# Zialus/CUDA-Recommender

Hardware: AMD Instinct MI355X
Metric: rating-nnz/sec per CCD++ outer iter at k=64 (higher is better)
Workload: dtype f32

## Files before the change

cuda-recommender_amd/csrc/ccd_kernels.hip:

```cpp
#include "ccd_kernels.hpp"

#include <algorithm>
#include <cstdlib>
#include <mutex>
#include <type_traits>

#include "flat_layout.hpp"

namespace mfx {
namespace {

constexpr int kBlock = 256;
constexpr uint32_t kPerSegLdsCap = 1024;

using u32x4 = __attribute__((ext_vector_type(4))) uint32_t;
using f32x4 = __attribute__((ext_vector_type(4))) float;
using u16x4 = __attribute__((ext_vector_type(4))) uint16_t;

template <int CTRL, int ROW_MASK = 0xF>
__device__ __forceinline__ float dpp_mov(float src) {
    return __builtin_bit_cast(float, __builtin_amdgcn_update_dpp(0, __builtin_bit_cast(int, src), CTRL, ROW_MASK, 0xF, true));
}
constexpr int kDppRowShr = 0x110, kDppWaveShr1 = 0x138, kDppBcast15 = 0x142, kDppBcast31 = 0x143;

// ... 111 lines not shown
    const uint32_t* orphans;
    uint32_t norphans, ngroups, panel_lanes;
    uint32_t nseg, npanels;
    const uint32_t* ptr_v;
    const uint32_t* rank_code;
    const uint32_t* seg_cnt;
    float lambda;
    float* out_vec;
    float2* pack2;
    const float* next_vec;
    float4* pack4;
    const float* gather_aux;
};

struct F3 { float x, y, z; };
template <typename S, typename G> __device__ __forceinline__ S to_slice(const G& g) { return g; }
template <> __device__ __forceinline__ F3 to_slice<F3, float4>(const float4& g) { return F3{g.x, g.y, g.z}; }
template <typename G, typename S> __device__ __forceinline__ G from_slice(const S& s) { return s; }
template <> __device__ __forceinline__ float4 from_slice<float4, F3>(const F3& s) { return make_float4(s.x, s.y, s.z, 0.f); }
template <int MODE> struct ModeTraits;
template <> struct ModeTraits<FM_SWEEP> { using G = float;  using S = float;  using P = float;  static constexpr bool kPerSeg = false, kWrite = false, kDot = true, kAux = false; };
template <> struct ModeTraits<FM_RESID> { using G = float;  using S = float;  using P = float;  static constexpr bool kPerSeg = true,  kWrite = true,  kDot = false, kAux = false; };
template <> struct ModeTraits<FM_FCSC>  { using G = float2; using S = float2; using P = float2; static constexpr bool kPerSeg = true,  kWrite = true,  kDot = true, kAux = false; };
template <> struct ModeTraits<FM_FCSR>  { using G = float4; using S = F3;     using P = float2; static constexpr bool kPerSeg = true,  kWrite = true,  kDot = true, kAux = false; };
template <> struct ModeTraits<FM_FCSC_RO> { using G = float2; using S = float2; using P = float2; static constexpr bool kPerSeg = true, kWrite = false, kDot = true, kAux = false; };
template <> struct ModeTraits<FM_FCSR_RO> { using G = float4; using S = F3;     using P = float2; static constexpr bool kPerSeg = true, kWrite = false, kDot = true, kAux = false; };
template <> struct ModeTraits<FM_FCSC2> { using G = float4; using S = float4; using P = float4; static constexpr bool kPerSeg = true,  kWrite = true,  kDot = true, kAux = false; };
template <> struct ModeTraits<FM_FCSR2> { using G = float4; using S = float4; using P = float4; static constexpr bool kPerSeg = true,  kWrite = true,  kDot = true, kAux = true; };

__device__ __forceinline__ float zero_of(float) { return 0.f; }
__device__ __forceinline__ float2 zero_of(float2) { return make_float2(0.f, 0.f); }
__device__ __forceinline__ float4 zero_of(float4) { return make_float4(0.f, 0.f, 0.f, 0.f); }

template <int MODE>
__device__ __forceinline__ void element_op(float v, const typename ModeTraits<MODE>::G& ga, float aux,
                                           const typename ModeTraits<MODE>::P& ps, int add,
                                           float& v_out, float& gc, float& hc) {
    if constexpr (MODE == FM_SWEEP) {
        v_out = v;
        gc = ga * v;
        hc = ga * ga;
    } else if constexpr (MODE == FM_RESID) {
        const float prod = mul_rn(ga, ps);
        v_out = add ? add_rn(v, prod) : sub_rn(v, prod);
        gc = 0.f;
        hc = 0.f;
    } else if constexpr (MODE == FM_FCSC || MODE == FM_FCSC_RO) {
        v_out = add_rn(sub_rn(v, mul_rn(ga.x, ps.x)), mul_rn(ga.y, ps.y));
        gc = ga.y * v_out;
        hc = ga.y * ga.y;
    } else if constexpr (MODE == FM_FCSR || MODE == FM_FCSR_RO) {
        v_out = add_rn(sub_rn(v, mul_rn(ga.x, ps.x)), mul_rn(ga.y, ps.y));
        gc = ga.z * v_out;
        hc = ga.z * ga.z;
    } else {
        const float r = add_rn(sub_rn(v, mul_rn(ga.x, ps.x)), mul_rn(ga.y, ps.y));
        v_out = add_rn(sub_rn(r, mul_rn(ga.z, ps.z)), mul_rn(ga.w, ps.w));
        const float d = MODE == FM_FCSC2 ? ga.w : aux;
        gc = d * v_out;
        hc = d * d;
    }
}

template <int BLOCK> __device__ void fused_finalize(const FlatArgs& a, uint32_t chunk, unsigned char* lds_raw);

using gu64 = __attribute__((address_space(1))) unsigned long long;
using gu32 = __attribute__((address_space(1))) uint32_t;
template <bool FUSE>
__device__ __forceinline__ void store_partial(float2* p, float g, float h) {
    if constexpr (FUSE) {
        const unsigned long long bits = (unsigned long long) __builtin_bit_cast(uint32_t, g) | ((unsigned long long) __builtin_bit_cast(uint32_t, h) << 32);
        __hip_atomic_store((gu64*) p, bits, __ATOMIC_RELAXED, __HIP_MEMORY_SCOPE_AGENT);
    } else {
        *p = make_float2(g, h);
    }
}
__device__ __forceinline__ float2 load_partial_sc1(const float2* p) {
    const unsigned long long bits = __hip_atomic_load((gu64*) p, __ATOMIC_RELAXED, __HIP_MEMORY_SCOPE_AGENT);
    return make_float2(__builtin_bit_cast(float, (uint32_t) bits), __builtin_bit_cast(float, (uint32_t) (bits >> 32)));
}

template <int MODE> constexpr int flat_min_waves(int block) { return MODE == FM_FCSC_RO || MODE == FM_FCSR_RO ? block / 128 : 1; }

template <int MODE, bool LDS, int BLOCK, bool PSCHK, bool FUSE = false, bool PERSIST = false>
__global__ __launch_bounds__(BLOCK, flat_min_waves<MODE>(BLOCK)) void k_flat(FlatArgs a) {
    static_assert(!FUSE || ModeTraits<MODE>::kDot, "fused finalize: passes that produce sums");
    static_assert(!PERSIST || (LDS && !FUSE), "persistent form: LDS panels without the in-pass finalize");
    using TR = ModeTraits<MODE>;
    uint32_t chunk = FUSE ? a.wg_order[blockIdx.x] : blockIdx.x;
    uint32_t chunk_end = chunk + 1;
    const uint32_t nchunks = a.nspans / (BLOCK / 64);
    if constexpr (PERSIST) {
        chunk = (uint32_t) ((uint64_t) blockIdx.x * nchunks / gridDim.x);
        chunk_end = (uint32_t) ((uint64_t) (blockIdx.x + 1) * nchunks / gridDim.x);
        if (chunk >= chunk_end) return;
    }
    using G = typename TR::G;
    using P = typename TR::P;
    extern __shared__ __attribute__((aligned(16))) unsigned char lds_raw[];
    using S = typename TR::S;
    S* __restrict__ slice = reinterpret_cast<S*>(lds_raw);
    constexpr size_t kSliceEntry = sizeof(S) + (TR::kAux ? sizeof(float) : 0);
    float* __restrict__ aux_slice = reinterpret_cast<float*>(lds_raw + ((size_t) a.panel_rows + 1) * sizeof(S));
    const uint32_t lane = threadIdx.x & 63;
    uint32_t span = __builtin_amdgcn_readfirstlane(chunk * (BLOCK / 64) + (threadIdx.x >> 6));
    const G* __restrict__ gather = static_cast<const G*>(a.gather);
    const P* __restrict__ perseg = static_cast<const P*>(a.perseg);
    const uint32_t span_words = a.tiles_per_span * (kTileElems / 32);
    uint64_t start = (uint64_t) span * a.tiles_per_span * kTileElems;
    using IdxVec = typename std::conditional<LDS, u16x4, u32x4>::type;
    using IdxElem = typename std::conditional<LDS, uint16_t, uint32_t>::type;
    const IdxVec* __restrict__ idx4 = reinterpret_cast<const IdxVec*>(static_cast<const IdxElem*>(a.idx) + start) + lane;
    f32x4* __restrict__ val4 = reinterpret_cast<f32x4*>(a.val + start) + lane;
    const uint32_t* __restrict__ flw = a.flags32 + (size_t) span * span_words + (lane >> 3);
    const uint32_t* __restrict__ hpw = a.hpre + (size_t) span * span_words + (lane >> 3);
    const uint32_t sh = (lane & 7) * 4;
    IdxVec id_n;
    f32x4 v_n;
    uint32_t fl_n, hp_n, hp_nn;
    const size_t span_step_q = (size_t) (BLOCK / 64) * a.tiles_per_span * 64, span_step_w = (size_t) (BLOCK / 64) * span_words;
    auto stage_slice = [&](uint32_t panel) {
        const uint32_t gbase = panel * a.panel_rows;
        const uint32_t cnt = a.gather_len - gbase < a.panel_rows ? a.gather_len - gbase : a.panel_rows;
        for (uint32_t i = threadIdx.x; i < cnt; i += BLOCK) slice[i] = to_slice<S, G>(gather[gbase + i]);
        if (threadIdx.x == 0) slice[a.panel_rows] = S{};
        if constexpr (TR::kAux) {
            for (uint32_t i = threadIdx.x; i < cnt; i += BLOCK) aux_slice[i] = a.gather_aux[gbase + i];
            if (threadIdx.x == 0) aux_slice[a.panel_rows] = 0.f;
        }
    };
    uint32_t panel = 0, panel_next = 0;
    if constexpr (LDS) {
        id_n = __builtin_nontemporal_load(idx4);
        v_n = __builtin_nontemporal_load(val4);
        fl_n = flw[0]; hp_n = hpw[0]; hp_nn = hpw[8];
        panel = a.wg_panel[chunk];
        stage_slice(panel);
    }
    P* __restrict__ ps_lds = reinterpret_cast<P*>(lds_raw + (((size_t) a.panel_rows + 1) * kSliceEntry + 15) / 16 * 16);
    uint32_t win_base = 0;
    auto heads_before = [&](uint32_t c) { return a.hpre[(size_t) c * (BLOCK / 64) * span_words]; };
    uint32_t hb1 = 0, hb2 = 0;
    if constexpr (LDS && TR::kPerSeg) {
        const uint32_t rb0 = heads_before(chunk);
        win_base = rb0 > 0 ? rb0 - 1 : 0;
        const uint32_t win_end = heads_before(chunk + 1);
        if constexpr (PERSIST) { hb1 = win_end; hb2 = heads_before(chunk + 2 < nchunks ? chunk + 2 : nchunks); }
        uint32_t cnt = win_end - win_base;
        if (cnt > kPerSegLdsCap) cnt = kPerSegLdsCap;
        for (uint32_t j = threadIdx.x; j < cnt; j += BLOCK) ps_lds[j] = perseg[a.seg_of_rank[win_base + j]];
    }
    if constexpr (LDS && !PERSIST) __syncthreads();
    for (uint32_t visit = 0;; ++visit) {
    const bool more = PERSIST && chunk + 1 < chunk_end;
    uint32_t win_base_n = 0, win_cnt_n = 0;
    if constexpr (PERSIST) {
        if (visit && panel_next != panel) {
            __syncthreads();
            panel = panel_next;
            stage_slice(panel);
        }
        __syncthreads();
        if constexpr (TR::kPerSeg) {
            if (more) {
                win_base_n = hb1 > 0 ? hb1 - 1 : 0;
                win_cnt_n = hb2 - win_base_n < kPerSegLdsCap ? hb2 - win_base_n : kPerSegLdsCap;
            }
        }
    }
    P* __restrict__ ps_cur = PERSIST ? ps_lds + (visit & 1u) * kPerSegLdsCap : ps_lds;
    bool live = span < a.nspans;
    if constexpr (!FUSE) { if (!live) return; }
    auto fetch_ps = [&](uint32_t r) -> P {
        if constexpr (LDS) {
            const uint32_t rl = r - win_base;
            if constexpr (!PSCHK) return ps_cur[rl];
            else if (rl < kPerSegLdsCap) return ps_cur[rl];
        }
        return perseg[a.seg_of_rank[r]];
    };
    uint32_t ntiles = a.tiles_per_span;
    if constexpr (!LDS) {
        const uint64_t left = a.nnz > start ? a.nnz - start : 0;
        const uint32_t nlive = (uint32_t) ((left + kTileElems - 1) / kTileElems);
        if (nlive < ntiles) ntiles = nlive;
        if (live && ntiles == 0) {
            if (TR::kDot && lane == 0) store_partial<FUSE>(a.carry + span, 0.f, 0.f);
            live = false;
        }
        if constexpr (!FUSE) { if (!live) return; }
        if (live) {
            id_n = __builtin_nontemporal_load(idx4);
            v_n = __builtin_nontemporal_load(val4);
            fl_n = flw[0]; hp_n = hpw[0]; hp_nn = hpw[8];
        }
    }
    if (live) {
    const uint32_t rank_base = __builtin_amdgcn_readfirstlane(hp_n);
    uint32_t cur1 = rank_base;
    P pcur{};
    if constexpr (TR::kPerSeg) {
        if (cur1 > 0) pcur = fetch_ps(cur1 - 1);
    }
    float og = 0.f, oh = 0.f;
    bool open_spread = false;

    for (uint32_t tile = 0; tile < ntiles; ++tile) {
        const IdxVec id = id_n;
        const f32x4 v = v_n;
        const uint32_t fl = fl_n, hp = hp_n;
        const uint32_t cur1_next = __builtin_amdgcn_readfirstlane(hp_nn);
        hp_n = hp_nn;
        if constexpr (!PERSIST) {
            if (tile + 1 < ntiles) {
                id_n = __builtin_nontemporal_load(idx4 + (tile + 1) * 64);
                v_n = __builtin_nontemporal_load(val4 + (tile + 1) * 64);
            }
            fl_n = flw[(tile + 1) * 8];
            hp_nn = hpw[(tile + 2) * 8];
        } else if (tile + 1 < ntiles) {
            id_n = __builtin_nontemporal_load(idx4 + (tile + 1) * 64);
            v_n = __builtin_nontemporal_load(val4 + (tile + 1) * 64);
            fl_n = flw[(tile + 1) * 8];
            hp_nn = hpw[(tile + 2) * 8];
        } else if (more) {
            id_n = __builtin_nontemporal_load(idx4 + span_step_q);
            v_n = __builtin_nontemporal_load(val4 + span_step_q);
            fl_n = flw[span_step_w]; hp_n = hpw[span_step_w]; hp_nn = hpw[span_step_w + 8];
            panel_next = a.wg_panel[chunk + 1];
            if constexpr (TR::kPerSeg) { hb1 = hb2; hb2 = heads_before(chunk + 3 < nchunks ? chunk + 3 : nchunks); }
        }
        const uint64_t base = start + (uint64_t) tile * kTileElems;
        const bool partial = !LDS && base + kTileElems > a.nnz;
        const uint64_t e0 = base + (uint64_t) lane * 4;

        const uint32_t ids[4] = {(uint32_t) id.x, (uint32_t) id.y, (uint32_t) id.z, (uint32_t) id.w};
        const float vs[4] = {v.x, v.y, v.z, v.w};
        G ga[4];
        float gx[4] = {};
#pragma unroll
        for (int e = 0; e < 4; ++e) {
            if constexpr (LDS) ga[e] = from_slice<G, S>(slice[ids[e]]);
            else ga[e] = ids[e] < a.gather_len ? gather[ids[e]] : zero_of(G{});
            if constexpr (LDS && TR::kAux) gx[e] = aux_slice[ids[e]];
        }
        float vo[4], gc[4], hc[4];

        if (cur1_next == cur1) {
#pragma unroll
            for (int e = 0; e < 4; ++e) {
                element_op<MODE>(vs[e], ga[e], gx[e], pcur, a.add, vo[e], gc[e], hc[e]);
                if (partial && e0 + e >= a.nnz) { gc[e] = 0.f; hc[e] = 0.f; }
                if constexpr (TR::kDot) { og += gc[e]; oh += hc[e]; }
            }
            open_spread = true;
        } else {
            const uint32_t nib = (fl >> sh) & 0xFu;
            const uint32_t r1 = hp + (uint32_t) __popc(fl & ((1u << sh) - 1u));
#pragma unroll
            for (int e = 0; e < 4; ++e) {
                P ps{};
                if constexpr (TR::kPerSeg) {
                    const uint32_t re1 = r1 + (uint32_t) __popc(nib & ((2u << e) - 1u));
                    ps = fetch_ps(re1 - 1);
                }
                element_op<MODE>(vs[e], ga[e], gx[e], ps, a.add, vo[e], gc[e], hc[e]);
                if (partial && e0 + e >= a.nnz) { gc[e] = 0.f; hc[e] = 0.f; }
            }
            if constexpr (TR::kDot) {
                float cin_g, cin_h;
                if (open_spread) {
                    cin_g = wave_sum(og);
                    cin_h = wave_sum(oh);
                } else {
                    cin_g = __builtin_bit_cast(float, __builtin_amdgcn_readfirstlane(__builtin_bit_cast(int, og)));
                    cin_h = __builtin_bit_cast(float, __builtin_amdgcn_readfirstlane(__builtin_bit_cast(int, oh)));
                }
                open_spread = false;
                float ag = 0.f, ah = 0.f, fg = 0.f, fh = 0.f;
                bool seen = false;
                uint32_t close1 = r1;
#pragma unroll
                for (int e = 0; e < 4; ++e) {
                    if ((nib >> e) & 1u) {
                        if (!seen) {
                            fg = ag; fh = ah; seen = true;
                        } else {
                            store_partial<FUSE>(a.part + (close1 - 1), ag, ah);
                        }
                        ++close1;
                        ag = 0.f; ah = 0.f;
                    }
                    ag += gc[e];
                    ah += hc[e];
                }
                if (!seen) { fg = ag; fh = ah; }
                const uint64_t M = __ballot(seen);
                const uint64_t upto = M & ((uint64_t(2) << lane) - 1);
                const uint32_t dist = upto ? lane - (63u - (uint32_t) __clzll((long long) upto)) : 64u;
                float xg = ag, xh = ah;
                seg_scan2(xg, xh, lane, dist);
                float eg = dpp_mov<kDppWaveShr1>(xg), eh = dpp_mov<kDppWaveShr1>(xh);
                if ((M & ((uint64_t(1) << lane) - 1)) == 0) { eg += cin_g; eh += cin_h; }
                if (seen) {
                    const float tg = eg + fg, th = eh + fh;
                    if (r1 > rank_base) {
                        store_partial<FUSE>(a.part + (r1 - 1), tg, th);
                    } else {
                        store_partial<FUSE>(a.carry + span, tg, th);
                    }
                }
                const float ng = __builtin_bit_cast(float, __builtin_amdgcn_readlane(__builtin_bit_cast(int, xg), 63));
                const float nh = __builtin_bit_cast(float, __builtin_amdgcn_readlane(__builtin_bit_cast(int, xh), 63));
                og = lane == 0 ? ng : 0.f;
                oh = lane == 0 ? nh : 0.f;
            }
            cur1 = cur1_next;
            if constexpr (TR::kPerSeg) pcur = fetch_ps(cur1 - 1);
        }
        if constexpr (TR::kWrite) {
            if (!partial) {
__builtin_nontemporal_store(f32x4{vo[0], vo[1], vo[2], vo[3]}, val4 + tile * 64);
            } else {
                float* vp = a.val + e0;
#pragma unroll
                for (int e = 0; e < 4; ++e)
                    if (e0 + e < a.nnz) vp[e] = vo[e];
            }
        }
    }
    if constexpr (TR::kDot) {
        const float tg = open_spread ? wave_sum(og) : og, th = open_spread ? wave_sum(oh) : oh;
        if (lane == 0) {
            if (cur1 > rank_base) {
                store_partial<FUSE>(a.part + (cur1 - 1), tg, th);
            } else {
                store_partial<FUSE>(a.carry + span, tg, th);
            }
        }
    }
    }
    if constexpr (!PERSIST) break;
    if (!more) break;
    if constexpr (TR::kPerSeg) {
        P* __restrict__ ps_nxt = ps_lds + ((visit + 1) & 1u) * kPerSegLdsCap;
        for (uint32_t j = threadIdx.x; j < win_cnt_n; j += BLOCK) ps_nxt[j] = perseg[a.seg_of_rank[win_base_n + j]];
        win_base = win_base_n;
    }
    ++chunk;
    span += BLOCK / 64;
    start = (uint64_t) span * a.tiles_per_span * kTileElems;
    idx4 = reinterpret_cast<const IdxVec*>(static_cast<const IdxElem*>(a.idx) + start) + lane;
    val4 = reinterpret_cast<f32x4*>(a.val + start) + lane;
    flw = a.flags32 + (size_t) span * span_words + (lane >> 3);
    hpw = a.hpre + (size_t) span * span_words + (lane >> 3);
    }
    if constexpr (FUSE) fused_finalize<BLOCK>(a, chunk, lds_raw);
}


constexpr uint32_t kSegOwnerLong = 1024;
#ifndef MFX_OWNER_UL
#define MFX_OWNER_UL 2
#define MFX_OWNER_US 1
#endif
#ifndef MFX_SEG_BLOCK
#define MFX_SEG_BLOCK 256
#endif
constexpr int kSegBlock = MFX_SEG_BLOCK;
struct SegOwnerArgs {
    const uint32_t* ptr;
    const uint32_t* idx;
    float* val;
    const void* gather;
    const void* perseg;
    const uint4* long_list;
    const uint4* short_list;
    uint32_t nlong, nshort;
    float lambda;
    float* out_vec;
    float2* pack2;
    const float* next_vec;
    float4* pack4;
};

template <int MODE>
__device__ __forceinline__ void seg_owner_finish(const SegOwnerArgs& a, uint32_t c, uint32_t cnt, float g, float h,
                                                 const typename ModeTraits<MODE>::P& ps, float next_old) {
    const float x = cnt ? g / add_rn(mul_rn(a.lambda, (float) cnt), h) : 0.f;
    a.out_vec[c] = x;
    if constexpr (MODE == FM_FCSC || MODE == FM_FCSR) {
        if (a.pack4) a.pack4[c] = make_float4(ps.x, ps.y, x, 0.f);
        a.pack2[c] = make_float2(x, a.next_vec == a.out_vec ? x : next_old);
    }
}

template <int MODE>
__global__ __launch_bounds__(kSegBlock) void k_seg_owner(SegOwnerArgs a) {
    using TR = ModeTraits<MODE>;
    using G = typename TR::G;
    using P = typename TR::P;
    const G* __restrict__ gather = static_cast<const G*>(a.gather);
    const P* __restrict__ perseg = static_cast<const P*>(a.perseg);
    const uint32_t lane = threadIdx.x & 63, wave = threadIdx.x >> 6;
    __shared__ float sg[kSegBlock / 64], sh[kSegBlock / 64];
    auto walk = [&](uint32_t lo, uint32_t hi, uint32_t first, uint32_t stride, const P& ps, float& g, float& h, auto unroll) {
        constexpr int U = decltype(unroll)::value;
        g = 0.f; h = 0.f;
        if (hi == lo) return;
        const uint32_t base = lo & ~3u;
        uint32_t pq[U];
        u32x4 id4[U];
        f32x4 v4[U];
        auto streams = [&](uint32_t p0, uint32_t (&pp)[U], u32x4 (&ii)[U], f32x4 (&vals)[U]) {
#pragma unroll
            for (int u = 0; u < U; ++u) {
                pp[u] = p0 + (uint32_t) u * 4u * stride;
                const uint32_t at = pp[u] < hi ? pp[u] : base;
                ii[u] = *reinterpret_cast<const u32x4*>(a.idx + at);
                vals[u] = *reinterpret_cast<const f32x4*>(a.val + at);
            }
        };
        uint32_t p = base + 4u * first;
        if (p < hi) streams(p, pq, id4, v4);
        while (p < hi) {
            G ga[U][4];
// ... 432 lines not shown
}

__global__ __launch_bounds__(kBlock) void k_chunk_seg_range(uint32_t nchunks, uint64_t chunk_len, const uint32_t* __restrict__ ptr_v,
                                                             size_t nv, uint32_t nseg, const uint32_t* __restrict__ wg_panel,
                                                             const uint32_t* __restrict__ panel_end, uint32_t* __restrict__ seg_first,
                                                             uint32_t* __restrict__ seg_last) {
    const uint32_t w = blockIdx.x * kBlock + threadIdx.x;
    if (w >= nchunks) return;
    const uint64_t lo = (uint64_t) w * chunk_len;
    uint64_t hi = lo + chunk_len;
    const uint32_t pe = panel_end[wg_panel ? wg_panel[w] : 0u];
    if (hi > pe) hi = pe;
    if (hi <= lo) { seg_first[w] = 0xFFFFFFFFu; seg_last[w] = 0; return; }
    auto holder = [&](uint32_t q) {
        size_t a = 0, b = nv;
        while (b - a > 1) {
            const size_t mid = a + (b - a) / 2;
            if (ptr_v[mid] <= q) a = mid; else b = mid;
        }
        return (uint32_t) (a % nseg);
    };
    seg_first[w] = holder((uint32_t) lo);
    seg_last[w] = holder((uint32_t) (hi - 1));
}

uint32_t seg_grid(uint32_t nseg) {
    const uint32_t want = (nseg + (kBlock / 64) - 1) / (kBlock / 64);
    return want < 1 ? 1 : (want > 256 * 8 ? 256 * 8 : want);
}

}

#define MFX_LAUNCH_CHECK() MFX_HIP(hipGetLastError())

namespace {
struct LdsAttrCache {
    std::mutex m;
    size_t bytes[64] = {};
};
int ensure_dynamic_lds(const void* kernel, LdsAttrCache& c, size_t lds_bytes) {
    int dev = 0;
    MFX_HIP(hipGetDevice(&dev));
    std::lock_guard<std::mutex> lk(c.m);
    if (dev >= 0 && dev < 64 && lds_bytes <= c.bytes[dev]) return MFX_OK;
    MFX_HIP(hipFuncSetAttribute(kernel, hipFuncAttributeMaxDynamicSharedMemorySize, (int) lds_bytes));
    if (dev >= 0 && dev < 64) c.bytes[dev] = lds_bytes;
    return MFX_OK;
}
}

template <int MODE, bool LDS, int BLOCK, bool PSCHK, bool FUSE = false, bool PERSIST = false>
int launch_flat_t(const FlatArgs& a, uint32_t grid, size_t lds_bytes, hipStream_t st) {
    if (lds_bytes > 48 * 1024) {
        static LdsAttrCache cache;
        MFX_TRY(ensure_dynamic_lds(reinterpret_cast<const void*>(k_flat<MODE, LDS, BLOCK, PSCHK, FUSE, PERSIST>), cache, lds_bytes));
    }
    hipLaunchKernelGGL((k_flat<MODE, LDS, BLOCK, PSCHK, FUSE, PERSIST>), dim3(grid), dim3(BLOCK), lds_bytes, st, a);
    MFX_LAUNCH_CHECK();
    return MFX_OK;
}

template <int MODE, int BLOCK, bool PSCHK>
uint32_t flat_persist_per_cu(size_t lds_bytes) {
    static std::mutex m;
    static int by_regs[64] = {};
    int dev = 0;
    if (hipGetDevice(&dev) != hipSuccess || dev < 0 || dev >= 64) dev = 0;
    std::lock_guard<std::mutex> lk(m);
    if (by_regs[dev] == 0) {
        int n = 0;
        if (hipOccupancyMaxActiveBlocksPerMultiprocessor(&n, reinterpret_cast<const void*>(k_flat<MODE, true, BLOCK, PSCHK, false, true>), BLOCK, 0) != hipSuccess || n < 1) {
            (void) hipGetLastError();
            n = 1;
        }
        by_regs[dev] = n;
    }
    const size_t by_lds = lds_bytes ? (size_t) 160 * 1024 / lds_bytes : 1;
    return (uint32_t) std::max<size_t>(1, std::min<size_t>((size_t) by_regs[dev], by_lds));
}

template <int MODE, int BLOCK, bool PSCHK>
int launch_flat_persist(const SegStreamDev& s, const FlatArgs& a, uint32_t grid, size_t lds_bytes, hipStream_t st) {
    if ((s.flat_persist_modes >> MODE) & 1u) {
        const size_t lds2 = lds_bytes + (size_t) kPerSegLdsCap * sizeof(typename ModeTraits<MODE>::P);
        if (lds2 <= 160 * 1024) {
            const uint32_t resident = s.flat_cus * flat_persist_per_cu<MODE, BLOCK, PSCHK>(lds2);
            const uint32_t g = s.flat_persist_wgs ? s.flat_persist_wgs : (grid / 2 >= resident ? resident : grid);
            if (g >= 1 && g < grid) return launch_flat_t<MODE, true, BLOCK, PSCHK, false, true>(a, g, lds2, st);
        }
    }
    return launch_flat_t<MODE, true, BLOCK, PSCHK>(a, grid, lds_bytes, st);
}

template <int MODE, int BLOCK>
int launch_flat_lds(const SegStreamDev& s, const FlatArgs& a, uint32_t grid, size_t lds_bytes, hipStream_t st) {
    if (ModeTraits<MODE>::kPerSeg && s.max_wg_ranks > kPerSegLdsCap)
        return launch_flat_t<MODE, true, BLOCK, true>(a, grid, lds_bytes, st);
    return launch_flat_t<MODE, true, BLOCK, false>(a, grid, lds_bytes, st);
}

template <int MODE>
int launch_flat_mode(const SegStreamDev& s, const FlatArgs& a, hipStream_t st) {
    if (!s.lds_panels)
        return launch_flat_t<MODE, false, kBlock, false>(a, (s.nspans + (kBlock / 64) - 1) / (kBlock / 64), 0, st);
    const size_t entry = sizeof(typename ModeTraits<MODE>::S) + (ModeTraits<MODE>::kAux ? sizeof(float) : 0);
    size_t lds_bytes = (((size_t) s.panel_rows + 1) * entry + 15) / 16 * 16;
    if (ModeTraits<MODE>::kPerSeg) lds_bytes += (size_t) kPerSegLdsCap * sizeof(typename ModeTraits<MODE>::P);
    const uint32_t grid = s.nspans / s.spans_per_wg;
    switch (s.spans_per_wg) {
        case 4: return launch_flat_lds<MODE, 256>(s, a, grid, lds_bytes, st);
        case 8: return launch_flat_lds<MODE, 512>(s, a, grid, lds_bytes, st);
        case 16: return launch_flat_lds<MODE, 1024>(s, a, grid, lds_bytes, st);
        default: return fail(MFX_ERR_INVALID, "panel layout: spans_per_wg must be 4, 8 or 16 (got %u)", s.spans_per_wg);
    }
}

static FlatArgs flat_args_of(const SegStreamDev& s, const void* gather, const void* perseg, int add) {
    FlatArgs a = {};
    a.idx = s.lds_panels ? static_cast<const void*>(s.idx16) : static_cast<const void*>(s.idx);
    a.val = s.val; a.flags32 = s.flags32; a.hpre = s.hpre; a.seg_of_rank = s.seg_of_rank;
    a.wg_panel = s.wg_panel; a.nspans = s.nspans;
    a.tiles_per_span = s.tiles_per_span; a.panel_rows = s.panel_rows; a.gather_len = s.gather_len; a.nne = s.nne;
    a.nnz = (s.panel_rows && !s.lds_panels) ? s.padded_nnz : s.nnz; a.gather = gather; a.perseg = perseg; a.part = s.part;
    a.carry = s.carry; a.add = add;
    return a;
}

static int panel_lanes(const SegStreamDev& s);
uint32_t fused_group_size(uint32_t npanels, uint32_t block) { return block / (npanels >= 8 ? 16u : npanels >= 2 ? 4u : 1u); }

template <int MODE>
int launch_flat_fused_mode(const SegStreamDev& s, const FlatArgs& a, hipStream_t st) {
    if (!s.panel_rows) {
        const size_t epilogue = 2 * kBlock * sizeof(float) + ((size_t) s.fz_max_chunk_groups + 2) * sizeof(uint32_t);
        return launch_flat_t<MODE, false, kBlock, false, true>(a, (s.nspans + (kBlock / 64) - 1) / (kBlock / 64), epilogue, st);
    }
    size_t lds_bytes = (((size_t) s.panel_rows + 1) * sizeof(typename ModeTraits<MODE>::S) + 15) / 16 * 16 + (size_t) kPerSegLdsCap * sizeof(typename ModeTraits<MODE>::P);
    const size_t epilogue = 2 * 1024 * sizeof(float) + ((size_t) s.fz_max_chunk_groups + 2) * sizeof(uint32_t);
    if (lds_bytes < epilogue) lds_bytes = epilogue;
    const uint32_t grid = s.nspans / s.spans_per_wg;
    if (s.max_wg_ranks > kPerSegLdsCap) return launch_flat_t<MODE, true, 1024, true, true>(a, grid, lds_bytes, st);
    return launch_flat_t<MODE, true, 1024, false, true>(a, grid, lds_bytes, st);
}

int launch_flat_fused(FlatMode mode, const SegStreamDev& s, const void* gather, const void* perseg, const FinalizeArgs& f, hipStream_t st) {
    MFX_REQUIRE(((s.lds_panels && s.spans_per_wg == 16) || !s.panel_rows) && s.fz_order && s.fz_g0 && s.fz_g1 && s.fz_expected && s.fz_arrived,
                "launch_flat_fused: the layout carries no fused-finalize tables");
    MFX_REQUIRE(!f.gh_dense && !f.cnt_override && !f.pack4_as3 && !f.nmf && !f.fundec_seg && !f.quad, "launch_flat_fused: dense / overridden / extended finalize inputs are not fused");
    MFX_REQUIRE(mode == FM_FCSC || mode == FM_FCSR || mode == FM_SWEEP, "launch_flat_fused: bad mode %d", (int) mode);
    FlatArgs a = flat_args_of(s, gather, perseg, 0);
    a.wg_order = s.fz_order; a.wg_g0 = s.fz_g0; a.wg_g1 = s.fz_g1; a.expected = s.fz_expected; a.arrived = s.fz_arrived;
    a.orphans = s.fz_orphans; a.norphans = s.fz_norphans; a.ngroups = s.fz_ngroups; a.panel_lanes = (uint32_t) panel_lanes(s);
    a.nseg = s.nseg; a.npanels = s.npanels; a.ptr_v = s.ptr_v; a.rank_code = s.rank_code; a.seg_cnt = s.seg_cnt;
    a.lambda = f.lambda; a.out_vec = f.out_vec; a.pack2 = f.pack2; a.next_vec = f.next_vec; a.pack4 = f.pack4;
    if (mode == FM_SWEEP) {
        MFX_REQUIRE(!s.panel_rows, "launch_flat_fused: the fused read-only sweep exists for the plain layout only");
        return launch_flat_fused_mode<FM_SWEEP>(s, a, st);
    }
    return mode == FM_FCSC ? launch_flat_fused_mode<FM_FCSC>(s, a, st) : launch_flat_fused_mode<FM_FCSR>(s, a, st);
}

template <int MODE>
int launch_flat_lds_only(const SegStreamDev& s, const FlatArgs& a, hipStream_t st) {
    MFX_REQUIRE(s.lds_panels && !s.scatter, "launch_flat: mode %d needs the LDS-panel layout", MODE);
    const size_t entry = sizeof(typename ModeTraits<MODE>::S) + (ModeTraits<MODE>::kAux ? sizeof(float) : 0);
    size_t lds_bytes = (((size_t) s.panel_rows + 1) * entry + 15) / 16 * 16 + (size_t) kPerSegLdsCap * sizeof(typename ModeTraits<MODE>::P);
    MFX_REQUIRE(lds_bytes <= 160 * 1024, "launch_flat: mode %d needs %zu bytes of LDS at %u panel rows", MODE, lds_bytes, s.panel_rows);
    const uint32_t grid = s.nspans / s.spans_per_wg;
    if constexpr (!ModeTraits<MODE>::kWrite) {
        switch (s.spans_per_wg) {
            case 4: return launch_flat_lds<MODE, 256>(s, a, grid, lds_bytes, st);
            case 8: return launch_flat_lds<MODE, 512>(s, a, grid, lds_bytes, st);
            case 16: return launch_flat_lds<MODE, 1024>(s, a, grid, lds_bytes, st);
            default: return fail(MFX_ERR_INVALID, "panel layout: spans_per_wg must be 4, 8 or 16 (got %u)", s.spans_per_wg);
        }
    } else {
        const bool pschk = s.max_wg_ranks > kPerSegLdsCap;
        switch (s.spans_per_wg) {
            case 4: return pschk ? launch_flat_persist<MODE, 256, true>(s, a, grid, lds_bytes, st) : launch_flat_persist<MODE, 256, false>(s, a, grid, lds_bytes, st);
            case 8: return pschk ? launch_flat_persist<MODE, 512, true>(s, a, grid, lds_bytes, st) : launch_flat_persist<MODE, 512, false>(s, a, grid, lds_bytes, st);
            case 16: return pschk ? launch_flat_persist<MODE, 1024, true>(s, a, grid, lds_bytes, st) : launch_flat_persist<MODE, 1024, false>(s, a, grid, lds_bytes, st);
            default: return fail(MFX_ERR_INVALID, "panel layout: spans_per_wg must be 4, 8 or 16 (got %u)", s.spans_per_wg);
        }
    }
}

int launch_flat(FlatMode mode, const SegStreamDev& s, const void* gather, const void* perseg, int add,
                hipStream_t st, const float* gather_aux) {
    FlatArgs a = flat_args_of(s, gather, perseg, add);
    a.gather_aux = gather_aux;
    switch (mode) {
        case FM_SWEEP: return launch_flat_mode<FM_SWEEP>(s, a, st);
        case FM_RESID: return launch_flat_mode<FM_RESID>(s, a, st);
        case FM_FCSC: return launch_flat_mode<FM_FCSC>(s, a, st);
        case FM_FCSR: return launch_flat_mode<FM_FCSR>(s, a, st);
        case FM_FCSC_RO: return launch_flat_lds_only<FM_FCSC_RO>(s, a, st);
        case FM_FCSR_RO: return launch_flat_lds_only<FM_FCSR_RO>(s, a, st);
        case FM_FCSC2: return launch_flat_lds_only<FM_FCSC2>(s, a, st);
        case FM_FCSR2:
            MFX_REQUIRE(gather_aux, "launch_flat: FM_FCSR2 needs its fifth operand");
            return launch_flat_lds_only<FM_FCSR2>(s, a, st);
        default: return fail(MFX_ERR_INVALID, "launch_flat: bad mode %d", (int) mode);
    }
}

int launch_chunk_seg_range(const SegStreamDev& s, uint32_t wg_spans, const uint32_t* panel_end, uint32_t* seg_first, uint32_t* seg_last, hipStream_t st) {
    const uint32_t nchunks = (s.nspans + wg_spans - 1) / wg_spans;
    if (nchunks == 0) return MFX_OK;
    hipLaunchKernelGGL(k_chunk_seg_range, dim3((nchunks + kBlock - 1) / kBlock), dim3(kBlock), 0, st, nchunks,
                       (uint64_t) s.tiles_per_span * kTileElems * wg_spans, s.ptr_v, (size_t) s.npanels * s.nseg, s.nseg, s.panel_rows ? s.wg_panel : nullptr,
                       panel_end, seg_first, seg_last);
    MFX_LAUNCH_CHECK();
    return MFX_OK;
}

int check_index_range(const uint32_t* d_idx, uint64_t n, uint32_t bound, const char* what, hipStream_t st) {
    if (n == 0) return MFX_OK;
    DevBuf<unsigned long long> flag;
    MFX_TRY(flag.alloc(1));
    MFX_HIP(hipMemsetAsync(flag.get(), 0xFF, sizeof(unsigned long long), st));
    const uint32_t grid = (uint32_t) std::min<uint64_t>((n + kBlock - 1) / kBlock, 256 * 8);
    hipLaunchKernelGGL(k_check_range, dim3(grid), dim3(kBlock), 0, st, n, d_idx, bound, flag.get());
    MFX_LAUNCH_CHECK();
    unsigned long long bad = ~0ull;
    MFX_HIP(hipMemcpyAsync(&bad, flag.get(), sizeof(bad), hipMemcpyDeviceToHost, st));
    MFX_HIP(hipStreamSynchronize(st));
    if (bad == ~0ull) return MFX_OK;
    uint32_t v = 0;
    MFX_HIP(hipMemcpy(&v, d_idx + bad, sizeof(v), hipMemcpyDeviceToHost));
    return fail(MFX_ERR_INVALID, "%s %u at position %llu is out of range [0, %u)", what, v, bad, bound);
}

int launch_sweep_wave(const SegStreamDev& s, const float* vec, float* g_dense, float* h_dense, hipStream_t st) {
    if (s.nseg == 0) return MFX_OK;
    MFX_REQUIRE(s.panel_rows == 0, "wave-per-segment kernels need the plain layout");
    hipLaunchKernelGGL(k_sweep_wave, dim3(seg_grid(s.nseg)), dim3(kBlock), 0, st, s.nseg, s.ptr, s.idx, s.val,
                       vec, g_dense, h_dense);
    MFX_LAUNCH_CHECK();
    return MFX_OK;
}

int launch_resid_wave(const SegStreamDev& s, const float* gathered, const float* per_seg, int add, hipStream_t st) {
    if (s.nseg == 0) return MFX_OK;
    MFX_REQUIRE(s.panel_rows == 0, "wave-per-segment kernels need the plain layout");
    hipLaunchKernelGGL(k_resid_wave, dim3(seg_grid(s.nseg)), dim3(kBlock), 0, st, s.nseg, s.ptr, s.idx, s.val,
                       gathered, per_seg, add);
    MFX_LAUNCH_CHECK();
    return MFX_OK;
}

static GatherPartsArgs parts_of(const SegStreamDev& s) {
    GatherPartsArgs g;
    g.nseg = s.nseg; g.npanels = s.npanels; g.span_len = s.tiles_per_span * kTileElems; g.ptr_v = s.ptr_v;
    g.rank_code = s.rank_code; g.part = s.part; g.carry = s.carry;
    return g;
}

static int panel_lanes(const SegStreamDev& s) { return s.npanels >= 8 ? 16 : s.npanels >= 2 ? 4 : 1; }

int launch_combine_dense(const SegStreamDev& s, float* gh, hipStream_t st) {
    if (s.nseg == 0) return MFX_OK;
    const GatherPartsArgs a = parts_of(s);
    const int pl = panel_lanes(s);
    const dim3 grid((s.nseg + kBlock / pl - 1) / (kBlock / pl)), block(kBlock);
    if (pl == 16) hipLaunchKernelGGL(k_combine_dense<16>, grid, block, 0, st, a, gh);
    else if (pl == 4) hipLaunchKernelGGL(k_combine_dense<4>, grid, block, 0, st, a, gh);
// ... 115 lines not shown
```

cuda-recommender_amd/csrc/ccd_solver.hip:

```cpp
#include "ccd_solver.hpp"
#include "layout_kernels.hpp"

#include <algorithm>
#include <atomic>
#include <chrono>
#include <cmath>
#include <cstdlib>
#include <exception>
#include <string>
#include <thread>

namespace mfx {

namespace {
struct PhaseTimer {
    bool on = getenv("MFX_SETUP_TIMING") != nullptr;
    std::chrono::steady_clock::time_point t = std::chrono::steady_clock::now();
    void lap(const char* what) {
        if (!on) return;
        const auto n = std::chrono::steady_clock::now();
        fprintf(stderr, "[mfx setup] %-28s %7.1f ms\n", what, std::chrono::duration<double, std::milli>(n - t).count());
        t = n;
    }
};
// ... 623 lines not shown
    if (!scatter_) overlap_groups_ = 1;
    overlap_groups_ = std::min(overlap_groups_, csr_.view.scat_ngroups);
    if (overlap_groups_ > 1) {
        MFX_HIP(hipStreamCreateWithFlags(&st2_, hipStreamNonBlocking));
        for (uint32_t g = 0; g < overlap_groups_; ++g) MFX_HIP(hipEventCreateWithFlags(&ev_grp_[g], hipEventDisableTiming));
        MFX_HIP(hipEventCreateWithFlags(&ev_join_, hipEventDisableTiming));
    }
    if (ref_order_) {
        const char* e = std::getenv("MFX_REF_FUSED");
        ref_fused_ = !(e && std::atoi(e) == 0);
        for (int side = 0; side < 2; ++side) {
            const SegStreamDev& v = side == 0 ? csc_.view : csr_.view;
            std::vector<uint32_t> ptr_h((size_t) v.nseg + 1), order;
            MFX_HIP(hipMemcpyAsync(ptr_h.data(), v.ptr, sizeof(uint32_t) * ptr_h.size(), hipMemcpyDeviceToHost, st_));
            MFX_HIP(hipStreamSynchronize(st_));
            (side == 0 ? ref_nlong_csc_ : ref_nlong_csr_) = ref_sweep_order(ptr_h.data(), v.nseg, &order, ref_fused_);
            DevBuf<uint32_t>& dst = side == 0 ? ref_order_csc_ : ref_order_csr_;
            MFX_TRY(dst.alloc(order.size()));
            MFX_TRY(dst.upload(order.data(), order.size(), MFX_HOST, st_));
            MFX_HIP(hipStreamSynchronize(st_));
        }
        if (ref_fused_) {
            prof_.enable(p->profile != 0);
            ref_streams_.main = st_;
            MFX_HIP(hipStreamCreateWithFlags(&ref_streams_.side, hipStreamNonBlocking));
            MFX_HIP(hipEventCreateWithFlags(&ref_streams_.fork, hipEventDisableTiming));
            MFX_HIP(hipEventCreateWithFlags(&ref_streams_.join, hipEventDisableTiming));
            MFX_TRY(ref_zero_cols_.alloc_zero(n_, st_));
        }
    }

    MFX_TRY(W_.alloc_zero((size_t) k_ * m_, st_));
    MFX_TRY(H_.alloc_zero((size_t) k_ * n_, st_));
    MFX_TRY(packA_.alloc_zero(m_, st_));
    MFX_TRY(packB_.alloc_zero(n_, st_));
    MFX_TRY(packC_.alloc_zero(n_, st_));
    MFX_TRY(gh_cols_.alloc_zero((size_t) 2 * n_, st_));
    MFX_TRY(gh_rows_.alloc_zero((size_t) 2 * m_, st_));

    if (shard && shard->comm) {
        MFX_REQUIRE(shard->global_col_nnz, "sharded solve needs global_col_nnz");
        comm_ = shard->comm;
        MFX_TRY(global_col_nnz_.alloc(n_));
        MFX_TRY(global_col_nnz_.upload(shard->global_col_nnz, n_, space, st_));
        global_test_nnz_ = shard->global_test_nnz;
    }
    nnz_test_ = T ? T->nnz : 0;
    if (!comm_) global_test_nnz_ = nnz_test_;
    if (nnz_test_ > 0) {
        MFX_REQUIRE(T->row && T->col && T->val, "null test array");
        MFX_TRY(t_row_.alloc(nnz_test_)); MFX_TRY(t_row_.upload(T->row, nnz_test_, space, st_));
        MFX_TRY(t_col_.alloc(nnz_test_)); MFX_TRY(t_col_.upload(T->col, nnz_test_, space, st_));
        MFX_TRY(t_val_.alloc(nnz_test_)); MFX_TRY(t_val_.upload(T->val, nnz_test_, space, st_));
        MFX_TRY(check_index_range(t_row_.get(), (uint64_t) nnz_test_, m_, "test-set row", st_));
        MFX_TRY(check_index_range(t_col_.get(), (uint64_t) nnz_test_, n_, "test-set column", st_));
    }
    MFX_TRY(rmse_partials_.alloc_zero(kRmseBlocks, st_));
    MFX_REQUIRE(p->eps >= 0.f && p->eps < 1.f, "eps must be in [0, 1)");
    ext_on_ = p->do_nmf != 0 || p->eps > 0.f || p->rank_trace != 0;
    if (p->eps > 0.f || p->rank_trace) MFX_REQUIRE(!comm_, "eps / rank_trace are not available in a sharded solve");
    MFX_REQUIRE(!ref_order_ || !(p->do_nmf || p->eps > 0.f), "do_nmf / eps are not available with kernel_variant = -1");
    if (p->eps > 0.f) {
        MFX_TRY(fundec_seg_.alloc_zero(std::max(m_, n_), st_));
        MFX_TRY(fundec_sum_.alloc_zero(1, st_));
    }
    if (p->rank_trace) {
        MFX_TRY(old_w_.alloc_zero(m_, st_));
        MFX_TRY(old_h_.alloc_zero(n_, st_));
        MFX_TRY(test_resid_.alloc_zero(nnz_test_ > 0 ? (size_t) nnz_test_ : 1, st_));
        MFX_TRY(r1_sum_.alloc_zero(1, st_));
        for (hipEvent_t& e : ev_rank_) MFX_HIP(hipEventCreate(&e));
    }
    {
        const char* e = std::getenv("MFX_DEFER_RESID");
        auto fits = [](const SegStreamDev& v, size_t entry) {
            return ((size_t) v.panel_rows + 1) * entry + 15 + 1024 * sizeof(float4) <= 160 * 1024;
        };
        defer_resid_ = !(e && std::atoi(e) == 0) && p->schedule == 1 && p->maxinneriter == 1 && p->kernel_variant == 1 && !scatter_ &&
                       !owner_mode_ && !ref_order_ && !comm_ && fuse_finalize_ == 0 && !ext_on_ && csc_.view.lds_panels && csr_.view.lds_panels &&
                       fits(csc_.view, sizeof(float4)) && fits(csr_.view, sizeof(float4) + sizeof(float)) && k_ >= 2;
        if (defer_resid_) MFX_TRY(packD_.alloc_zero(m_, st_));
    }
    {
        uint32_t modes = (1u << FM_FCSC2) | (1u << FM_FCSR2);
        if (const char* e = std::getenv("MFX_FLAT_PERSIST")) { const long v = std::strtol(e, nullptr, 0); if (v == 0) modes = 0; else if (v > 1) modes &= (uint32_t) v; }
        uint32_t wgs = 0;
        if (const char* e = std::getenv("MFX_FLAT_WGS")) { const int v = std::atoi(e); if (v > 0) wgs = (uint32_t) v; }
        int dev = 0, cus = 0;
        MFX_HIP(hipGetDevice(&dev));
        MFX_HIP(hipDeviceGetAttribute(&cus, hipDeviceAttributeMultiprocessorCount, dev));
        for (SegStreamDev* v : {&csc_.view, &csr_.view}) {
            v->flat_persist_modes = defer_resid_ && cus > 0 ? modes : 0u;
            v->flat_cus = cus > 0 ? (uint32_t) cus : 0u;
            v->flat_persist_wgs = wgs;
        }
    }
    MFX_TRY(rmse_sum_.alloc_zero(1, st_));
    MFX_HIP(hipStreamSynchronize(st_));
    return MFX_OK;
}

int CcdSolver::build_stores(const mfx_csx* R, const mfx_params* p, mfx_memspace space, bool scatter) {
    const bool need_plain = p->schedule == 0 && p->kernel_variant <= 0;
    auto options = [&](uint32_t nseg, uint32_t G, uint32_t elem_bytes, bool is_csr) {
        if (!scatter) return choose_layout(*p, nseg, nnz_, G, elem_bytes, need_plain);
        constexpr uint32_t kScatterPanel = 6816;
        FlatLayoutOptions o;
        o.scatter = true; o.lds = true; o.spans_per_wg = 16;
        o.scatter_ids32 = p->kernel_variant == 3;
        o.panel_rows = std::min<uint32_t>(p->panel_rows > 0 ? (uint32_t) p->panel_rows : kScatterPanel, std::max<uint32_t>(G, 1u));
        const uint32_t groups = is_csr ? overlap_groups_ : 1u;
        o.scatter_groups = groups;
        int dev = 0, cus = 0;
        const char* mult_env = std::getenv("MFX_SCATTER_PANEL_MULT");
        const bool align = !(mult_env && std::atoi(mult_env) == 0);
        if (p->panel_rows == 0 && hipGetDevice(&dev) == hipSuccess &&
            hipDeviceGetAttribute(&cus, hipDeviceAttributeMultiprocessorCount, dev) == hipSuccess && cus >= 16) {
            uint32_t nwg = (uint32_t) cus;
            if (is_csr && comm_reserve_cus_ > 0 && comm_reserve_cus_ + 8 <= nwg) { nwg = (nwg - comm_reserve_cus_) / 8 * 8; o.scatter_wgs = nwg; }
            const uint32_t q = nwg / 8, p0 = (G + kScatterPanel - 1) / kScatterPanel;
            auto gcd = [](uint32_t a, uint32_t b) { while (b) { const uint32_t t = a % b; a = b; b = t; } return a; };
            uint32_t P = 0;
            if (align && p0 >= q / 2 * groups) {
                for (uint32_t c = (p0 + groups - 1) / groups * groups; c <= 2 * p0 + q * groups; c += groups)
                    if (q / gcd(q, c / groups) <= 2) { P = c; break; }
            }
            if (P == 0 && groups > 1 && p0 >= groups) P = (p0 + groups - 1) / groups * groups;
            if (P == 0 && align && p0 > 1) P = p0;
            if (P) o.panel_rows = (G + P - 1) / P;
        }
        o.tiles_per_span = p->tiles_per_span > 0 ? (uint32_t) p->tiles_per_span : (nnz_ >= (32u << 20) ? 4u : 0u);
        return o;
    };
    scatter_ = scatter;
    int rc_csr = MFX_OK;
    std::string err_csr;
    ThreadGang csr_gang;
    csr_gang.run([&] {
        try {
            rc_csr = use_device(device_);
            if (rc_csr == MFX_OK)
                rc_csr = csr_.build(m_, nnz_, n_, R->csr_row_ptr, R->csr_col_idx, R->csr_val, space, options(m_, n_, kCsrSliceBytes, true),
                                    scatter ? 2 : p->layout_build, st_);
        } catch (const std::exception& ex) {
            rc_csr = fail(MFX_ERR_ALLOC, "building the CSR copy failed: %s", ex.what());
        }
        if (rc_csr != MFX_OK) err_csr = last_error();
    });
    int rc_csc;
    try {
        rc_csc = csc_.build(n_, nnz_, m_, R->csc_col_ptr, R->csc_row_idx, R->csc_val, space, options(n_, m_, sizeof(float2), false),
                            scatter ? 2 : p->layout_build, st_);
    } catch (const std::exception& ex) {
        rc_csc = fail(MFX_ERR_ALLOC, "building the CSC copy failed: %s", ex.what());
    }
    csr_gang.wait();
    if (rc_csc != MFX_OK) return rc_csc;
    if (rc_csr != MFX_OK) { last_error() = err_csr; return rc_csr; }
    return MFX_OK;
}

int CcdSolver::set_factors(const float* W, const float* H, mfx_memspace space) {
    MFX_REQUIRE(W, "mfx_ccd_set_factors: W is required");
    MFX_REQUIRE(oiter_ == 0, "factors can only be set before the first iteration");
    MFX_REQUIRE(H == nullptr, "mfx_ccd_set_factors: H must be NULL (CCD++ starts from H = 0)");
    MFX_TRY(use_device(device_));
    MFX_TRY(W_.upload(W, (size_t) k_ * m_, space, st_));
// ... 547 lines not shown
```

Baseline: 4.550 billion.

## Run read-only flat passes as persistent workgroups with scalar-base prefetch

Extends the persistent-workgroup form to the read-only FCSC_RO/FCSR_RO passes, enabled by default. Each resident workgroup walks a contiguous range of chunks, restaging the LDS panel only when it changes and reloading the per-segment window between chunks without double buffering. Prefetch loads use readfirstlane-uniform base pointers plus per-lane offsets so the compiler can use scalar bases. The intent is to cut launch and tail overhead and repeated panel staging, at the cost of extra barriers per chunk and lower occupancy if LDS use limits residency.

```diff
diff --git a/cuda-recommender_amd/csrc/ccd_kernels.hip b/cuda-recommender_amd/csrc/ccd_kernels.hip
--- a/cuda-recommender_amd/csrc/ccd_kernels.hip
+++ b/cuda-recommender_amd/csrc/ccd_kernels.hip
@@ -217,11 +217,16 @@
 
 template <int MODE> constexpr int flat_min_waves(int block) { return MODE == FM_FCSC_RO || MODE == FM_FCSR_RO ? block / 128 : 1; }
 
+#ifndef MFX_RO_PERSIST_FORM
+#define MFX_RO_PERSIST_FORM 1
+#endif
 template <int MODE, bool LDS, int BLOCK, bool PSCHK, bool FUSE = false, bool PERSIST = false>
 __global__ __launch_bounds__(BLOCK, flat_min_waves<MODE>(BLOCK)) void k_flat(FlatArgs a) {
     static_assert(!FUSE || ModeTraits<MODE>::kDot, "fused finalize: passes that produce sums");
     static_assert(!PERSIST || (LDS && !FUSE), "persistent form: LDS panels without the in-pass finalize");
     using TR = ModeTraits<MODE>;
+    constexpr bool ROP = PERSIST && !TR::kWrite;
+    constexpr bool PERSIST2 = PERSIST && TR::kWrite;
     uint32_t chunk = FUSE ? a.wg_order[blockIdx.x] : blockIdx.x;
     uint32_t chunk_end = chunk + 1;
     const uint32_t nchunks = a.nspans / (BLOCK / 64);
@@ -254,6 +259,20 @@
     f32x4 v_n;
     uint32_t fl_n, hp_n, hp_nn;
     const size_t span_step_q = (size_t) (BLOCK / 64) * a.tiles_per_span * 64, span_step_w = (size_t) (BLOCK / 64) * span_words;
+    uint64_t sq = ROP ? (uint64_t) span * a.tiles_per_span * 64 : 0, sw = ROP ? (uint64_t) span * span_words : 0;
+    struct LaneOff { uint32_t i, v, w; };
+    auto lane_off = [](uint32_t lane) { LaneOff o{lane * (uint32_t) sizeof(IdxVec), lane * 16u, (lane >> 3) * 4u}; asm volatile("" : "+v"(o.i), "+v"(o.v), "+v"(o.w)); return o; };
+    using gchar = __attribute__((address_space(1))) const char;
+    auto ubase = [](const void* p) {
+        const uint64_t u = reinterpret_cast<uint64_t>(p);
+        return reinterpret_cast<gchar*>((uint64_t) (uint32_t) __builtin_amdgcn_readfirstlane((int) (u >> 32)) << 32 | (uint32_t) __builtin_amdgcn_readfirstlane((int) u));
+    };
+    using GIdxVec = __attribute__((address_space(1))) const IdxVec;
+    using GF32x4 = __attribute__((address_space(1))) const f32x4;
+    auto ld_idx = [&](uint64_t q, uint32_t lane_ib) { return __builtin_nontemporal_load(reinterpret_cast<GIdxVec*>(ubase(static_cast<const IdxVec*>(a.idx) + (sq + q)) + lane_ib)); };
+    auto ld_val = [&](uint64_t q, uint32_t lane_vb) { return __builtin_nontemporal_load(reinterpret_cast<GF32x4*>(ubase(reinterpret_cast<const f32x4*>(a.val) + (sq + q)) + lane_vb)); };
+    auto ld_fl = [&](uint64_t w, uint32_t lane_wb) { return *reinterpret_cast<const gu32*>(ubase(a.flags32 + (sw + w)) + lane_wb); };
+    auto ld_hp = [&](uint64_t w, uint32_t lane_wb) { return *reinterpret_cast<const gu32*>(ubase(a.hpre + (sw + w)) + lane_wb); };
     auto stage_slice = [&](uint32_t panel) {
         const uint32_t gbase = panel * a.panel_rows;
         const uint32_t cnt = a.gather_len - gbase < a.panel_rows ? a.gather_len - gbase : a.panel_rows;
@@ -280,7 +299,7 @@
         const uint32_t rb0 = heads_before(chunk);
         win_base = rb0 > 0 ? rb0 - 1 : 0;
         const uint32_t win_end = heads_before(chunk + 1);
-        if constexpr (PERSIST) { hb1 = win_end; hb2 = heads_before(chunk + 2 < nchunks ? chunk + 2 : nchunks); }
+        if constexpr (PERSIST2) { hb1 = win_end; hb2 = heads_before(chunk + 2 < nchunks ? chunk + 2 : nchunks); }
         uint32_t cnt = win_end - win_base;
         if (cnt > kPerSegLdsCap) cnt = kPerSegLdsCap;
         for (uint32_t j = threadIdx.x; j < cnt; j += BLOCK) ps_lds[j] = perseg[a.seg_of_rank[win_base + j]];
@@ -289,7 +308,8 @@
     for (uint32_t visit = 0;; ++visit) {
     const bool more = PERSIST && chunk + 1 < chunk_end;
     uint32_t win_base_n = 0, win_cnt_n = 0;
-    if constexpr (PERSIST) {
+    if constexpr (ROP) __syncthreads();
+    if constexpr (PERSIST2) {
         if (visit && panel_next != panel) {
             __syncthreads();
             panel = panel_next;
@@ -303,7 +323,7 @@
             }
         }
     }
-    P* __restrict__ ps_cur = PERSIST ? ps_lds + (visit & 1u) * kPerSegLdsCap : ps_lds;
+    P* __restrict__ ps_cur = PERSIST2 ? ps_lds + (visit & 1u) * kPerSegLdsCap : ps_lds;
     bool live = span < a.nspans;
     if constexpr (!FUSE) { if (!live) return; }
     auto fetch_ps = [&](uint32_t r) -> P {
@@ -346,7 +366,18 @@
         const uint32_t fl = fl_n, hp = hp_n;
         const uint32_t cur1_next = __builtin_amdgcn_readfirstlane(hp_nn);
         hp_n = hp_nn;
-        if constexpr (!PERSIST) {
+        if constexpr (ROP) {
+            const bool hop = MFX_RO_PERSIST_FORM == 2 && more && tile + 1 == ntiles;
+            const uint64_t q = hop ? (uint64_t) span_step_q : (uint64_t) (tile + 1) * 64;
+            const uint64_t w = hop ? (uint64_t) span_step_w : (uint64_t) (tile + 1) * 8;
+            const LaneOff lo = lane_off(lane);
+            if (hop || tile + 1 < ntiles) {
+                id_n = ld_idx(q, lo.i);
+                v_n = ld_val(q, lo.v);
+            }
+            fl_n = ld_fl(w, lo.w);
+            hp_nn = ld_hp(w + 8, lo.w);
+        } else if constexpr (!PERSIST) {
             if (tile + 1 < ntiles) {
                 id_n = __builtin_nontemporal_load(idx4 + (tile + 1) * 64);
                 v_n = __builtin_nontemporal_load(val4 + (tile + 1) * 64);
@@ -477,6 +508,30 @@
     }
     if constexpr (!PERSIST) break;
     if (!more) break;
+    if constexpr (ROP) {
+        ++chunk;
+        span += BLOCK / 64;
+        sq += span_step_q;
+        sw += span_step_w;
+        const LaneOff lo = lane_off(lane);
+        if (MFX_RO_PERSIST_FORM != 2) {
+            id_n = ld_idx(0, lo.i);
+            v_n = ld_val(0, lo.v);
+            fl_n = ld_fl(0, lo.w); hp_nn = ld_hp(8, lo.w);
+        }
+        hp_n = ld_hp(0, lo.w);
+        panel_next = a.wg_panel[chunk];
+        const uint32_t rb0 = heads_before(chunk), win_end = heads_before(chunk + 1);
+        __syncthreads();
+        if (panel_next != panel) {
+            panel = panel_next;
+            stage_slice(panel);
+        }
+        win_base = rb0 > 0 ? rb0 - 1 : 0;
+        const uint32_t cnt = win_end - win_base < kPerSegLdsCap ? win_end - win_base : kPerSegLdsCap;
+        for (uint32_t j = threadIdx.x; j < cnt; j += BLOCK) ps_lds[j] = perseg[a.seg_of_rank[win_base + j]];
+        continue;
+    }
     if constexpr (TR::kPerSeg) {
         P* __restrict__ ps_nxt = ps_lds + ((visit + 1) & 1u) * kPerSegLdsCap;
         for (uint32_t j = threadIdx.x; j < win_cnt_n; j += BLOCK) ps_nxt[j] = perseg[a.seg_of_rank[win_base_n + j]];
@@ -1075,7 +1130,7 @@
 template <int MODE, int BLOCK, bool PSCHK>
 int launch_flat_persist(const SegStreamDev& s, const FlatArgs& a, uint32_t grid, size_t lds_bytes, hipStream_t st) {
     if ((s.flat_persist_modes >> MODE) & 1u) {
-        const size_t lds2 = lds_bytes + (size_t) kPerSegLdsCap * sizeof(typename ModeTraits<MODE>::P);
+        const size_t lds2 = lds_bytes + (ModeTraits<MODE>::kWrite ? (size_t) kPerSegLdsCap * sizeof(typename ModeTraits<MODE>::P) : 0);
         if (lds2 <= 160 * 1024) {
             const uint32_t resident = s.flat_cus * flat_persist_per_cu<MODE, BLOCK, PSCHK>(lds2);
             const uint32_t g = s.flat_persist_wgs ? s.flat_persist_wgs : (grid / 2 >= resident ? resident : grid);
@@ -1160,21 +1215,12 @@
     size_t lds_bytes = (((size_t) s.panel_rows + 1) * entry + 15) / 16 * 16 + (size_t) kPerSegLdsCap * sizeof(typename ModeTraits<MODE>::P);
     MFX_REQUIRE(lds_bytes <= 160 * 1024, "launch_flat: mode %d needs %zu bytes of LDS at %u panel rows", MODE, lds_bytes, s.panel_rows);
     const uint32_t grid = s.nspans / s.spans_per_wg;
-    if constexpr (!ModeTraits<MODE>::kWrite) {
-        switch (s.spans_per_wg) {
-            case 4: return launch_flat_lds<MODE, 256>(s, a, grid, lds_bytes, st);
-            case 8: return launch_flat_lds<MODE, 512>(s, a, grid, lds_bytes, st);
-            case 16: return launch_flat_lds<MODE, 1024>(s, a, grid, lds_bytes, st);
-            default: return fail(MFX_ERR_INVALID, "panel layout: spans_per_wg must be 4, 8 or 16 (got %u)", s.spans_per_wg);
-        }
-    } else {
-        const bool pschk = s.max_wg_ranks > kPerSegLdsCap;
-        switch (s.spans_per_wg) {
-            case 4: return pschk ? launch_flat_persist<MODE, 256, true>(s, a, grid, lds_bytes, st) : launch_flat_persist<MODE, 256, false>(s, a, grid, lds_bytes, st);
-            case 8: return pschk ? launch_flat_persist<MODE, 512, true>(s, a, grid, lds_bytes, st) : launch_flat_persist<MODE, 512, false>(s, a, grid, lds_bytes, st);
-            case 16: return pschk ? launch_flat_persist<MODE, 1024, true>(s, a, grid, lds_bytes, st) : launch_flat_persist<MODE, 1024, false>(s, a, grid, lds_bytes, st);
-            default: return fail(MFX_ERR_INVALID, "panel layout: spans_per_wg must be 4, 8 or 16 (got %u)", s.spans_per_wg);
-        }
+    const bool pschk = s.max_wg_ranks > kPerSegLdsCap;
+    switch (s.spans_per_wg) {
+        case 4: return pschk ? launch_flat_persist<MODE, 256, true>(s, a, grid, lds_bytes, st) : launch_flat_persist<MODE, 256, false>(s, a, grid, lds_bytes, st);
+        case 8: return pschk ? launch_flat_persist<MODE, 512, true>(s, a, grid, lds_bytes, st) : launch_flat_persist<MODE, 512, false>(s, a, grid, lds_bytes, st);
+        case 16: return pschk ? launch_flat_persist<MODE, 1024, true>(s, a, grid, lds_bytes, st) : launch_flat_persist<MODE, 1024, false>(s, a, grid, lds_bytes, st);
+        default: return fail(MFX_ERR_INVALID, "panel layout: spans_per_wg must be 4, 8 or 16 (got %u)", s.spans_per_wg);
     }
 }
 
diff --git a/cuda-recommender_amd/csrc/ccd_solver.hip b/cuda-recommender_amd/csrc/ccd_solver.hip
--- a/cuda-recommender_amd/csrc/ccd_solver.hip
+++ b/cuda-recommender_amd/csrc/ccd_solver.hip
@@ -729,7 +729,7 @@
         if (defer_resid_) MFX_TRY(packD_.alloc_zero(m_, st_));
     }
     {
-        uint32_t modes = (1u << FM_FCSC2) | (1u << FM_FCSR2);
+        uint32_t modes = (1u << FM_FCSC_RO) | (1u << FM_FCSR_RO) | (1u << FM_FCSC2) | (1u << FM_FCSR2);
         if (const char* e = std::getenv("MFX_FLAT_PERSIST")) { const long v = std::strtol(e, nullptr, 0); if (v == 0) modes = 0; else if (v > 1) modes &= (uint32_t) v; }
         uint32_t wgs = 0;
         if (const char* e = std::getenv("MFX_FLAT_WGS")) { const int v = std::atoi(e); if (v > 0) wgs = (uint32_t) v; }
```

New measurement: 4.657 billion, median of 6. +2.4%, better.
